# ishine/Prior-DiffuSE

Measured on AMD Instinct MI355X. Metric: enhanced-audio sec/sec (RTF), 6-step fast sampling, B=32, higher is better.
Workload: dtype f16x2; 1 GPU; B=32 x 4 s 16 kHz utterances per GPU, [B,2,401,161] spectrograms, GCRN prior + DiffUNet1 6-step sampling, STFT..ISTFT, seeded random weights; global_batch=32, frames=401, parallelism=batch-shard x1, graph=True, streams_per_gpu=1, batches_in_flight=3

## Files before the change

prior-diffuse_amd/csrc/gconv4.hip:

```cpp
#include <hip/hip_runtime.h>
#include <stdint.h>
#include <stdio.h>
#include <stdlib.h>

#include "pdse.h"
#include "pdse_internal.h"

#include "gconv_common.h"

#ifndef G4_CH
#define G4_CH 3
#endif

__device__ __forceinline__ void glds16_g4(const void* g, void* l) {
  __builtin_amdgcn_global_load_lds((const __attribute__((address_space(1))) void*)g, (__attribute__((address_space(3))) void*)l,
                                   16, 0, 0);
}

__device__ __forceinline__ float g4_load(const float* sbase, const unsigned byte_off) {
  float v;
  asm volatile("global_load_dword %0, %1, %2" : "=v"(v) : "v"(byte_off), "s"(sbase) : "memory");
  return v;
}
typedef float g4_f32x4 __attribute__((ext_vector_type(4)));
__device__ __forceinline__ g4_f32x4 g4_load16(const float* sbase, const unsigned byte_off) {
  g4_f32x4 v;
  asm volatile("global_load_dwordx4 %0, %1, %2" : "=v"(v) : "v"(byte_off), "s"(sbase) : "memory");
  return v;
}
template <bool BLK>
struct g4_raw {
  float v[G4_CH][8];
  __device__ __forceinline__ float get(const int i, const int e) const { return v[i][e]; }
};
template <>
struct g4_raw<true> {
  g4_f32x4 v[G4_CH][2];
  __device__ __forceinline__ float get(const int i, const int e) const { return v[i][e >> 2][e & 3]; }
};
__device__ __forceinline__ void g4_landed(g4_raw<false>& raw) {
#pragma unroll
  for (int i = 0; i < G4_CH; ++i)
#pragma unroll
    for (int e = 0; e < 8; ++e) asm volatile("" : "+v"(raw.v[i][e]));
}
__device__ __forceinline__ void g4_landed(g4_raw<true>& raw) {
#pragma unroll
  for (int i = 0; i < G4_CH; ++i)
#pragma unroll
    for (int e = 0; e < 2; ++e) asm volatile("" : "+v"(raw.v[i][e]));
}

typedef unsigned u32x4 __attribute__((ext_vector_type(4)));
__device__ __forceinline__ void g4_lds_read3(const unsigned addr, u32x4 (&a)[3]) {
  asm volatile("ds_read_b128 %0, %3\n\tds_read_b128 %1, %3 offset:1024\n\tds_read_b128 %2, %3 offset:2048"
               : "=&v"(a[0]), "=&v"(a[1]), "=&v"(a[2])
               : "v"(addr)
               : "memory");
}
__device__ __forceinline__ void g4_lds_read3(const unsigned addr, u32x4 (&a)[2]) {
  asm volatile("ds_read_b128 %0, %2\n\tds_read_b128 %1, %2 offset:1024" : "=&v"(a[0]), "=&v"(a[1]) : "v"(addr) : "memory");
}
__device__ __forceinline__ void g4_lds_read3(const unsigned addr, u32x4 (&a)[1]) {
  asm volatile("ds_read_b128 %0, %1" : "=&v"(a[0]) : "v"(addr) : "memory");
}
template <int N, int NP>
__device__ __forceinline__ void g4_lds_wait(u32x4 (&a)[N][NP]) {
  asm volatile("s_waitcnt lgkmcnt(0)" ::: "memory");
#pragma unroll
  for (int i = 0; i < N; ++i)
#pragma unroll
    for (int p = 0; p < NP; ++p) asm volatile("" : "+v"(a[i][p]));
}
__device__ __forceinline__ f32x16 g4_mfma6(const u32x4 (&a)[3], const uint4 (&b)[3], f32x16 acc) {
  const uint4 a1 = make_uint4(a[0][0], a[0][1], a[0][2], a[0][3]), a2 = make_uint4(a[1][0], a[1][1], a[1][2], a[1][3]),
              a3 = make_uint4(a[2][0], a[2][1], a[2][2], a[2][3]);
  acc = mfma_bf16(a1, b[2], acc);
  acc = mfma_bf16(a3, b[0], acc);
  acc = mfma_bf16(a2, b[1], acc);
  acc = mfma_bf16(a1, b[1], acc);
  acc = mfma_bf16(a2, b[0], acc);
  acc = mfma_bf16(a1, b[0], acc);
  return acc;
}
__device__ __forceinline__ f32x16 g4_mfma6(const u32x4 (&a)[2], const uint4 (&b)[2], f32x16 acc) {
  const uint4 a1 = make_uint4(a[0][0], a[0][1], a[0][2], a[0][3]), a2 = make_uint4(a[1][0], a[1][1], a[1][2], a[1][3]);
  acc = mfma_f16(a2, b[0], acc);
  acc = mfma_f16(a1, b[1], acc);
  acc = mfma_f16(a1, b[0], acc);
  return acc;
}
__device__ __forceinline__ f32x16 g4_mfma6(const u32x4 (&a)[1], const uint4 (&b)[1], f32x16 acc) {
  return mfma_bf16(make_uint4(a[0][0], a[0][1], a[0][2], a[0][3]), b[0], acc);
}
__device__ __forceinline__ uint32_t g4_pack_bf16(const float a, const float b) {
  typedef float f32x2 __attribute__((ext_vector_type(2)));
  typedef __bf16 bf16x2 __attribute__((ext_vector_type(2)));
  const f32x2 v = {a, b};
  union { bf16x2 h; uint32_t u; } c;
  c.h = __builtin_convertvector(v, bf16x2);
  return c.u;
}
__device__ __forceinline__ void g4_split(const float (&x)[8], uint4 (&b)[3]) { split8(x, b[0], b[1], b[2]); }
__device__ __forceinline__ void g4_split(const float (&x)[8], uint4 (&b)[2]) { split8h(x, pow2i(PDSE_F16_ACT_EXP), b[0], b[1]); }
__device__ __forceinline__ void g4_split(const float (&x)[8], uint4 (&b)[1]) {
  b[0] = make_uint4(g4_pack_bf16(x[0], x[1]), g4_pack_bf16(x[2], x[3]), g4_pack_bf16(x[4], x[5]), g4_pack_bf16(x[6], x[7]));
}

struct g4_chunk {
  int s, tap, cb0, n, kb0;
};

__device__ long long* g_trace4 = nullptr;

template <int EPI, int MT, bool BLK, int NP = 3>
__global__ __launch_bounds__(512, 2) void gconv4_kernel(const pdse_gconv_desc d) {
  constexpr int FB = 64 * NP;
#ifdef PDSE_DIAG
  long long* const trace = g_trace4;
#else
  long long* const trace = nullptr;
#endif
  const long long c_start = trace ? clock64() : 0;
  long long c_req = 0, c_cmp = 0, c_bar = 0;
  constexpr bool DUAL = (EPI != PDSE_EPI_LINEAR);
  constexpr int NBR = DUAL ? 2 : 1, FR = NBR * MT;
  extern __shared__ uint4 ring[];
  const unsigned ring_base = (unsigned)(uintptr_t)ring;
  const int tid = threadIdx.x;
  const int lane = tid & 63, wave = tid >> 6;
  const int col = lane & 31, h = lane >> 5;
// ... 156 lines not shown
#pragma unroll
      for (int r = 0; r < 16; ++r) {
        acc0[m][r] *= us;
        if (DUAL) acc1[m][r] *= us;
      }
  }
  gconv_epilogue<EPI, MT>(d, tail_from_desc(d), acc0, acc1, b, t, j, pvalid, lane, h, mt0, mtiles);
  if (trace && lane == 0) {
    long long* q = trace + ((size_t)((blockIdx.z * gridDim.y + blockIdx.y) * gridDim.x + blockIdx.x) * 8 + wave) * 8;
    q[0] = c_pro - c_start;
    q[1] = c_req;
    q[2] = c_cmp;
    q[3] = c_bar;
    q[4] = nch;
    q[5] = clock64() - c_loop;
    q[6] = clock64() - c_start;
  }
}

template <int EPI, int MT, bool BLK, int NP>
static int launch4b(const pdse_gconv_desc* d, hipStream_t s, const int mtiles) {
  const int P = d->Tout * d->Fout;
  const dim3 grid(((P + 31) / 32 + 7) / 8, d->B, (mtiles + MT - 1) / MT), block(512);
  constexpr int FR = (EPI == PDSE_EPI_LINEAR ? 1 : 2) * MT;
  const size_t lds = (size_t)2 * G4_CH * FR * 64 * NP * sizeof(uint4);
  static unsigned long long attr_mask = 0;
  if (lds > 64 * 1024 && pdse_lds_attr((const void*)gconv4_kernel<EPI, MT, BLK, NP>, &attr_mask, "gconv4 lds attribute")) return 1;
  static const bool tracing = PDSE_DIAG_ENV("PDSE_G4_TRACE") != nullptr;
  static long long* tbuf = nullptr;
  const size_t nw = (size_t)grid.x * grid.y * grid.z * 8;
  if (tracing) {
    if (!tbuf) {
      (void)hipMalloc(&tbuf, (size_t)1 << 24);
      (void)hipMemcpyToSymbol(HIP_SYMBOL(g_trace4), &tbuf, sizeof(tbuf));
    }
    (void)hipMemsetAsync(tbuf, 0, nw * 64, s);
  }
  hipLaunchKernelGGL((gconv4_kernel<EPI, MT, BLK, NP>), grid, block, lds, s, *d);
  if (tracing && nw * 64 <= ((size_t)1 << 24)) {
    (void)hipStreamSynchronize(s);
    long long* h = (long long*)malloc(nw * 64);
    (void)hipMemcpy(h, tbuf, nw * 64, hipMemcpyDeviceToHost);
    double sum[7] = {0};
    for (size_t i = 0; i < nw; ++i)
      for (int k = 0; k < 7; ++k) sum[k] += (double)h[i * 8 + k];
    fprintf(stderr, "gconv4 trace EPI %d MT %d taps %d cin %d+%d cout %d %dx%d grid %ux%ux%u: prologue %.0f | per chunk: request %.0f compute %.0f barrier %.0f | chunks %.1f | epilogue %.0f total %.0f\n",
            EPI, MT, d->ntaps, d->in0.C, d->in1.C, d->Cout, d->Tout, d->Fout, grid.x, grid.y, grid.z, sum[0] / nw, sum[1] / sum[4], sum[2] / sum[4], sum[3] / sum[4],
            sum[4] / nw, sum[5] / nw, sum[6] / nw);
    free(h);
  }
  return pdse_check_launch("gconv4");
}

template <int EPI, int MT>
static int launch4(const pdse_gconv_desc* d, hipStream_t s, const int mtiles) {
  if (d->korder == 5)
    return d->in0.blk ? launch4b<EPI, MT, true, 2>(d, s, mtiles) : launch4b<EPI, MT, false, 2>(d, s, mtiles);
  if (d->korder == 4)
    return d->in0.blk ? launch4b<EPI, MT, true, 1>(d, s, mtiles) : launch4b<EPI, MT, false, 1>(d, s, mtiles);
  return d->in0.blk ? launch4b<EPI, MT, true, 3>(d, s, mtiles) : launch4b<EPI, MT, false, 3>(d, s, mtiles);
}

static int check4(const pdse_gconv_desc* d) {
  const bool two = d->in1.C > 0;
  const long long span0 = 4 * ((long long)d->B * d->in0.sb + 40ll * d->in0.sc), span1 = two ? 4 * ((long long)d->B * d->in1.sb + 40ll * d->in1.sc) : 0;
  auto blk_ok = [](const pdse_src& x) {
    return x.blk == 0 || (x.blk == 8 && !((x.sb | x.sc | x.st | x.sf) & 3) && (reinterpret_cast<uintptr_t>(x.ptr) & 15) == 0);
  };
  if (!blk_ok(d->in0) || (two && !blk_ok(d->in1)) || (two && d->in0.blk != d->in1.blk)) {
    pdse_set_error("gconv4: a channel-blocked source has blk = 8, strides in multiples of 4 floats and a 16-byte aligned base; "
                   "two sources are both blocked or both plain");
    return 1;
  }
  if (!(d->epi == PDSE_EPI_LINEAR || d->epi == PDSE_EPI_GLU) || (d->in0.C & 15) || (d->in1.C & 15) || d->in0.C == 0 || d->cin1 ||
      d->xf_mode != 0 || d->padrow != nullptr || d->ntaps > 12 || span0 >= (1ll << 32) || span1 >= (1ll << 32) ||
      (d->epi == PDSE_EPI_GLU && !d->w1) || (d->korder == 5 && (d->wexp < -40 || d->wexp > 40))) {
    pdse_set_error("gconv4: split-bf16 GEMM convolutions need LINEAR / GLU, channel counts in multiples of 16, <= 12 taps, "
                   "no load transform / pad row, 32-bit gather offsets");
    return 1;
  }
  return 0;
}

int pdse_gconv4_launch(const pdse_gconv_desc* d, hipStream_t s) {
  if (check4(d)) return 1;
  const int mtiles = (d->Cout + 31) / 32;
  if (d->epi == PDSE_EPI_GLU) return mtiles >= 2 ? launch4<PDSE_EPI_GLU, 2>(d, s, mtiles) : launch4<PDSE_EPI_GLU, 1>(d, s, mtiles);
  if (mtiles >= 4) return launch4<PDSE_EPI_LINEAR, 4>(d, s, mtiles);
  if (mtiles >= 2) return launch4<PDSE_EPI_LINEAR, 2>(d, s, mtiles);
  return launch4<PDSE_EPI_LINEAR, 1>(d, s, mtiles);
}

template <int MT, bool BLK>
__global__ __launch_bounds__(512, 2) void gconv4_pair_kernel(const pdse_gconv_desc d, const pdse_gconv_desc e) {
  constexpr int NP = 2, FB = 64 * NP;
  constexpr int FR = 2 * MT, FR2 = 2 * FR;
  extern __shared__ uint4 ring[];
  const unsigned ring_base = (unsigned)(uintptr_t)ring;
  const int tid = threadIdx.x;
  const int lane = tid & 63, wave = tid >> 6;
  const int col = lane & 31, h = lane >> 5;
  const int b = blockIdx.y;
  const int P = d.Tout * d.Fout;
  const int p = (blockIdx.x * 8 + wave) * 32 + col;
  const bool pvalid = p < P;
  const int t = pvalid ? p / d.Fout : 0;
  const int j = pvalid ? p - t * d.Fout : 0;
  const int mtiles = (d.Cout + 31) >> 5;
  const int mt0 = blockIdx.z * MT;

  const int cbn0 = d.in0.C >> 4, cbn1 = d.in1.C >> 4;
  const int cps0 = (cbn0 + G4_CH - 1) / G4_CH, cps1 = (cbn1 + G4_CH - 1) / G4_CH;
  const int nch0 = d.ntaps * cps0, nch = nch0 + d.ntaps * cps1;

  auto uni = [](const int v) { return __builtin_amdgcn_readfirstlane(v); };
  auto decode = [&](const int ci) {
    g4_chunk c;
    c.s = uni(ci >= nch0);
    const int q = c.s ? ci - nch0 : ci, cps = c.s ? cps1 : cps0, cbn = c.s ? cbn1 : cbn0;
    c.tap = uni(q / cps);
    c.cb0 = uni((q - c.tap * cps) * G4_CH);
    c.n = uni(min(G4_CH, cbn - c.cb0));
    c.kb0 = uni((c.s ? d.ntaps * cbn0 : 0) + c.tap * cbn + c.cb0);
    return c;
  };
  auto dma = [&](const g4_chunk& c, const int buf) {
    const int nf = c.tap == 0 ? FR2 : FR;
    const int kb1 = (c.s ? cbn0 : 0) + c.cb0;
    const int npieces = c.n * nf * NP;
    for (int pc = __builtin_amdgcn_readfirstlane(wave); pc < npieces; pc += 8) {
      const int i = pc / (nf * NP), rem = pc - i * (nf * NP), f = rem / NP, part = rem - f * NP;
      const bool odd = f >= FR;
      const int g = odd ? f - FR : f, br = g / MT, m = g - br * MT;
      if (mt0 + m < mtiles) {
        const float* const w = odd ? (br ? e.w1 : e.w0) : (br ? d.w1 : d.w0);
        const uint4* src = reinterpret_cast<const uint4*>(w) + ((size_t)((odd ? kb1 : c.kb0) + i) * mtiles + mt0 + m) * FB + part * 64 + lane;
        glds16_g4(src, ring + ((buf * G4_CH + i) * FR2 + f) * FB + part * 64);
      }
    }
  };
  auto gather = [&](const g4_chunk& c, g4_raw<BLK>& raw, bool& inb) {
    const bool s1 = c.s != 0;
    const float* const sptr = s1 ? d.in1.ptr : d.in0.ptr;
    const int64_t ssb = s1 ? d.in1.sb : d.in0.sb, ssc = s1 ? d.in1.sc : d.in0.sc, sst = s1 ? d.in1.st : d.in0.st,
                  ssf = s1 ? d.in1.sf : d.in0.sf;
    int dt = 0, df = 0;
#pragma unroll
    for (int k = 0; k < 12; ++k) {
      dt = c.tap == k ? d.tap_dt[k] : dt;
      df = c.tap == k ? d.tap_df[k] : df;
    }
    const int tin = t + dt, fin = j * d.sf_in + df;
    inb = pvalid && fin >= 0 && fin < d.Fin && tin >= 0 && tin < d.Tin;
    if constexpr (BLK) {
      const unsigned off = 4u * (unsigned)((inb ? (int64_t)b * ssb + (int64_t)tin * sst + (int64_t)fin * ssf : 0) + (int64_t)h * ssc);
#pragma unroll
      for (int i = 0; i < G4_CH; ++i) {
        if (i < c.n) {
          const float* base = sptr + (int64_t)(2 * (c.cb0 + i)) * ssc;
          raw.v[i][0] = g4_load16(base, off);
          raw.v[i][1] = g4_load16(base + 4, off);
        }
      }
    } else {
      const unsigned off = 4u * (unsigned)((inb ? (int64_t)b * ssb + (int64_t)tin * sst + (int64_t)fin * ssf : 0) + (int64_t)(8 * h) * ssc);
#pragma unroll
      for (int i = 0; i < G4_CH; ++i) {
        if (i < c.n) {
          const float* base = sptr + (int64_t)(16 * (c.cb0 + i)) * ssc;
// ... 130 lines not shown
```

prior-diffuse_amd/nets.py:

```python
import ctypes as C

import numpy as np
import torch

from . import _lib as L
from . import packing as P

F0 = 161
BIG = 1 << 30

TAG_NONE, TAG_EPS_BLOCK, TAG_EPS_CONV1, TAG_TCM, TAG_PRIOR, TAG_LSTM, TAG_SIGNAL, TAG_EW = range(8)


class WeightBank:

    def __init__(self):
        self.items = {}
        self.keep = []
        self.owners = []

    def token(self, obj):
        if obj is None:
            return None
        for i, o in enumerate(self.owners):
# ... 154 lines not shown
        f["wlc"], f["wrc"] = up16(P.pack_s3_chain(chain["wlc"])), up16(P.pack_s3_chain(chain["wrc"]))
        f["blc"], f["brc"], f["bc2"] = up(chain["blc"]), up(chain["brc"]), up(chain["bc2"])
        f["wc2"] = up(np.asarray(chain["wc2"], np.float64).reshape(32)) if chain["C2"] == 1 else up16(P.pack_s3_chain(chain["wc2"]))
        nx = w.get("nx")
        if nx:
            for i, tl in enumerate(nx):
                if tl.get("bias") is not None:
                    f[("nx_bias", i)] = up(tl["bias"])
            f["nx_w"] = up16(np.stack([P.pack_s3_chain(tl["w"])[0] for tl in nx], 0))
        return f

    def _gconv_weights_s3g(self, w, ntaps, c0, c1):
        ctx = self.ctx
        up = lambda a: ctx.up(a).data_ptr()
        up16 = lambda a: ctx.up(np.ascontiguousarray(a).view(np.int16), np.int16).data_ptr()
        npl = self.gemm_planes
        qe = P.f16_wexp(*[w[k_] for k_ in ("wk0", "wk1") if w.get(k_) is not None]) if npl == 2 else 0
        f = {"korder": {3: 3, 1: 4, 2: 5}[npl], "ksteps": ntaps * (c0 + c1) // 2, "w0": up16(P.pack_s3_gemm(w["wk0"], ntaps, c0, c1, npl, qe)),
             "wexp": qe}
        if w.get("wk1") is not None:
            f["w1"] = up16(P.pack_s3_gemm(w["wk1"], ntaps, c0, c1, npl, qe))
        for k in ("bias0", "bias1"):
            if w.get(k) is not None:
                f[k] = up(w[k])
        if w.get("post") is not None:
            f["post_scale"], f["post_shift"] = up(w["post"][0]), up(w["post"][1])
        return f

    def _gconv_weights(self, w, ntaps, c0, c1, epi, cin1, pipelined_ok):
        ctx = self.ctx
        up = lambda a: ctx.up(a).data_ptr()
        f = {}
        xf = w.get("xf")
        xf_mode = 0
        if xf is not None:
            xf_mode = f["xf_mode"] = xf["mode"]
            f["xf_scale0"], f["xf_shift0"], f["xf_slope0"] = up(xf["scale0"]), up(xf["shift0"]), float(xf["slope0"])
            if xf["mode"] == 2:
                f["xf_scale1"], f["xf_shift1"], f["xf_slope1"] = up(xf["scale1"]), up(xf["shift1"]), float(xf["slope1"])
        wk0 = np.asarray(w["wk0"])
        wk1 = w.get("wk1")
        key = (epi, ntaps, c1 > 0, xf_mode)
        if P.v2_supported(*key, cin1) and pipelined_ok:
            rows = P.korder1_rows(ntaps, c0, c1, P.V2_CP[key])
            f["w0"], f["ksteps"], f["korder"] = up(P.pack_a4(wk0, rows)), len(rows) // 2, 1
            if wk1 is not None:
                f["w1"] = up(P.pack_a4(wk1, rows))
            if w.get("wk2") is not None:
                rows1 = P.korder1_rows(w["ntaps1"], c0, 0, P.V2_CP[key])
                f["w2"], f["w3"] = up(P.pack_a4(w["wk2"], rows1)), up(P.pack_a4(w["wk3"], rows1))
                f["ksteps1"] = len(rows1) // 2
        else:
            w0 = P.pack_a(wk0)
            f["w0"], f["ksteps"] = up(w0), w0.shape[1]
            if wk1 is not None:
                f["w1"] = up(P.pack_a(wk1))
        for k in ("bias0", "bias1"):
            if w.get(k) is not None:
                f[k] = up(w[k])
        if w.get("post") is not None:
            f["post_scale"], f["post_shift"] = up(w["post"][0]), up(w["post"][1])
        chain = w.get("chain")
        if chain is not None:
            f["C2"] = chain["C2"]
            f["wlc"], f["wrc"] = up(P.pack_chain(chain["wlc"])), up(P.pack_chain(chain["wrc"]))
            f["blc"], f["brc"] = up(chain["blc"]), up(chain["brc"])
            f["wc2"] = up(np.asarray(chain["wc2"], np.float64).reshape(32)) if chain["C2"] == 1 else up(P.pack_chain(chain["wc2"]))
            f["bc2"] = up(chain["bc2"])
        nx = w.get("nx")
        if nx:
            packs = []
            for i, tl in enumerate(nx):
                wn = np.asarray(tl["w"], np.float64)
                packs.append(np.concatenate([P.pack_chain(wn[:, :32]), P.pack_chain(wn[:, 32:])], 0))
                if tl.get("bias") is not None:
                    f[("nx_bias", i)] = up(tl["bias"])
            f["nx_w"] = up(np.stack(packs, 0))
        return f

    def gconv(self, *, in0, in1=None, Tin, Fin, taps, sf_in, W, Cout, bias0=None, bias0_sb=0,
              bias1=None, bias1_sb=0, epi=L.EPI_LINEAR, act=L.ACT_NONE, act_slope=0.0,
              padrow=None, padrow_sb=0, padrow_off=0, cin1=False, resid=None, out,
              out_strides, out_off=0, out_cr=1, B, Tout, Fout, tag=TAG_NONE, bias0_off=0, phase1=None, nx=None,
              bias1_off=0, bias_t0=None, label="gconv", s3=False, s3g=False, has_xf=False):
        ctx = self.ctx
        d = L.GconvDesc()
        d.in0 = in0
        d.in1 = in1 if in1 is not None else L.Src(0, 0, 0, 0, 0, 0, 0)
        d.Tin, d.Fin = Tin, Fin
        d.padrow, d.padrow_sb = Ctx.ptr(padrow, padrow_off), padrow_sb
        ttaps = tuple((int(a), int(b)) for a, b in taps)
        tkey = ("taps", ttaps)
        tp = ctx.bank.items.get(tkey)
        if tp is None:
            ctx._banking += 1
            tp = ctx.bank.items[tkey] = ctx.up(P.taps_array(ttaps), np.int32)
            ctx._banking -= 1
        d.taps, d.ntaps, d.sf_in = tp.data_ptr(), len(ttaps), sf_in
        for i, (dt_, df_) in enumerate(ttaps[:12]):
            d.tap_dt[i], d.tap_df[i] = dt_, df_
        d.cin1 = 1 if cin1 else 0
        c0, c1 = d.in0.C, d.in1.C
        pipelined_ok = padrow is None and not self.force_generic
        s3 = bool(s3) and pipelined_ok and epi == L.EPI_BIGLU and (
            ((c0, c1) == (32, 0) and len(ttaps) in (4, 6)) or ((c0, c1, len(ttaps)) == (2, 2, 10) and phase1 is None))
        s3g = (bool(s3g) and not s3 and pipelined_ok and epi in (L.EPI_LINEAR, L.EPI_GLU) and not cin1 and not has_xf
               and c0 > 0 and c0 % 16 == 0 and c1 % 16 == 0 and len(ttaps) <= 12)
        site = "%s:%d:%d:%d:%d:%d:%d:%d:%d" % (label, epi, len(ttaps), c0, c1, Cout, pipelined_ok, s3, s3g)
        if s3g:
            f = self.memo(site, lambda: self._gconv_weights_s3g(W(), len(ttaps), c0, c1))
        elif s3:
            f = self.memo(site, lambda: self._gconv_weights_s3(W(), len(ttaps), c0 + c1))
        else:
            f = self.memo(site, lambda: self._gconv_weights(W(), len(ttaps), c0, c1, epi, cin1, pipelined_ok))
        for k, v in f.items():
            if isinstance(k, tuple):
                d.nx_bias[k[1]] = v
            else:
                setattr(d, k, v)
        d.Cout = Cout
        if bias0 is not None:
            d.bias0 = Ctx.ptr(bias0, bias0_off)
        if bias1 is not None:
            d.bias1 = Ctx.ptr(bias1, bias1_off)
        d.bias0_sb, d.bias1_sb = bias0_sb, bias1_sb
        if bias_t0 is not None:
            d.bias0_t0, d.bias1_t0 = Ctx.ptr(bias_t0[0], bias_t0[1]), Ctx.ptr(bias_t0[0], bias_t0[2])
        d.epi, d.act, d.act_slope = epi, act, float(act_slope)
        if phase1 is not None and d.korder in (1, 2):
            d.p1mask, d.Fout1 = phase1["mask"], phase1["Fout1"]
        elif phase1 is not None and d.korder == 5 and epi == L.EPI_GLU:
            d.p1mask, d.Fout1 = phase1["mask"], phase1["Fout1"]
        if nx is not None:
            tiles = nx["tiles"]
            d.nx_n, d.nx_keep, d.nx_row0 = len(tiles), 1 if nx.get("keep") else 0, nx.get("row0", -1)
            for i, tl in enumerate(tiles):
                if tl.get("bias") is not None:
                    d.nx_bias[i] = Ctx.ptr(tl["bias"], tl.get("bias_off", 0))
                d.nx_bias_sb[i] = tl.get("bias_sb", 0)
                d.nx_out[i] = Ctx.ptr(tl["out"])
                d.nx_sb[i], d.nx_sc[i], d.nx_st[i], d.nx_sf[i] = tl["strides"]
                d.nx_off[i] = tl.get("off", 0)
                d.nx_add[i] = Ctx.ptr(tl.get("add"))
        d.resid = Ctx.ptr(resid)
        d.out = Ctx.ptr(out)
        d.out_sb, d.out_sc_hi, d.out_sc_lo, d.out_st, d.out_sf = out_strides
        d.out_off, d.out_cr = out_off, out_cr
        d.B, d.Tout, d.Fout = B, Tout, Fout
        self.add(d, tag)
        return d


def nchw(C_, T, F):
    return C_ * T * F, T * F, F, 1


def nchw_out(C_, T, F):
    return C_ * T * F, T * F, 0, F, 1


def nc8(C_, T, F):
    return C_ * T * F, T * F * 8, F * 8, 8


def nc8_out(C_, T, F):
    return C_ * T * F, T * F * 8, 1, F * 8, 8


class EpsNetPlan(PlanBase):

    ENC_F = [161, 79, 39, 19, 9, 4]
    fused_tcm = True
    chain_conv1 = True
    compose_stage1 = True
    split_bf16 = True
    split_tcm = True
    plane_h = True
    tcm_stack = True
    parity_planes = True
    planes = 2
    TCM_F16 = True
    NSLOT = 20

    def __init__(self, ctx, sd, B, T, time_cond=True, nsteps=1, plan=None, table=None, with_pre=None, split_bf16=None,
                 planes=None, plane_h=None, exclusive=False, frames=None):
        with_pre = time_cond if with_pre is None else with_pre
        if split_bf16 is not None:
            self.split_bf16 = bool(split_bf16)
        if planes is not None:
            if int(planes) not in (1, 2, 3):
                raise ValueError("planes is 3 (bf16x3), 2 (f16x2) or 1 (bf16 mode)")
            self.planes = int(planes)
        if plane_h is not None:
            self.plane_h = bool(plane_h)
        if self.planes == 1:
            self.plane_h = True
        self.tcm_planes = 3 if (self.planes == 2 and not self.TCM_F16) else self.planes
        self.use_tcm_stack = bool(self.tcm_stack and exclusive)
        self.frames = frames
        if frames is not None and (self.force_generic or not self.fused_tcm):
            raise ValueError("exact ragged batches need a fused TCM form (csrc/tcm.hip, csrc/tcm2.hip): the three-launch form has no frames table")
        self.sd = sd
        ok = (self.split_bf16 and self.chain_conv1 and self.compose_stage1 and time_cond and with_pre and not self.force_generic
              and all(float(P._np(sd[k])[0]) <= 1.0 for k in sd if k.endswith(".weight") and P._np(sd[k]).shape == (1,)))
        if not ok:
            if self.planes == 1:
                raise ValueError("bf16 mode needs the chained split-bf16 DiffUNet1 path (PReLU slopes <= 1)")
            self.plane_h = False
            if self.planes == 2:
                self.planes = self.tcm_planes = 3
        super().__init__(ctx, plan, ns=(ctx.bank.token(sd), bool(time_cond), bool(with_pre), self.fused_tcm, self.chain_conv1,
                                        self.compose_stage1, self.split_bf16, self.split_tcm,
                                        ctx.bank.token(table), str(self.plane_h), self.planes, self.parity_planes))
        self.sd, self.B, self.T, self.time_cond, self.nsteps = sd, B, T, time_cond, nsteps
        self.with_pre = with_pre
# ... 622 lines not shown
                nx = dict(keep=False, row0=0, tiles=tiles)
            if chained and k == 1 and self.compose_stage1:
                Fin = self._biconvglu_composed(step, src_x, src_i, o, ostr, nx)
            else:
                Fin = self._biconvglu(step, k, src_x, src_i, Fin, o, ostr, H=Hc, do_conv1=(k == 1 or not chained), nx=nx)
            if chained:
                Hc, Hn = Hn, Hc
            src_x, src_i = self.src(o, 64, *nchw(64, T, Fin)), None
        cur, nxt = self.en[4], self.tcm_a
        names = [("TCMs.%d.residual%d" % (i, j + 1), dil) for i in range(3) for j, dil in enumerate((1, 2, 4, 8, 16, 32))]
        if self.force_generic or not self.fused_tcm:
            for p, dil in names:
                self._residual(p, dil, cur, nxt)
                cur, nxt = nxt, (self.tcm_b if nxt is self.tcm_a else self.tcm_a)
        elif self.split_bf16 and self.split_tcm:
            hcur, hnxt = self.tcm_hs
            self._residual_split(None, 1, cur, None, None, hcur, names[0][0], mode=1)
            self._tcm_stack = [] if self.use_tcm_stack else None
            for n, (p, dil) in enumerate(names):
                p_next = names[n + 1][0] if n + 1 < len(names) else None
                self._residual_split(p, dil, cur, nxt, hcur, hnxt, p_next)
                cur, nxt = nxt, (self.tcm_b if nxt is self.tcm_a else self.tcm_a)
                hcur, hnxt = hnxt, hcur
            if self._tcm_stack:
                sd_ = L.Tcm2sDesc()
                for n, blk in enumerate(self._tcm_stack):
                    sd_.blk[n] = blk
                sd_.n = len(self._tcm_stack)
                sd_.flags, sd_.status = self.tcm_flags.data_ptr(), self.tcm_status.data_ptr()
                self.add(sd_, TAG_TCM)
            self._tcm_stack = None
        else:
            hcur, hnxt = self.tcm_h, self.tcm_g
            self._tcm_conv1(names[0][0], cur, hcur)
            for n, (p, dil) in enumerate(names):
                p_next = names[n + 1][0] if n + 1 < len(names) else None
                self._residual_fused(p, dil, cur, nxt, hcur, hnxt, p_next)
                cur, nxt = nxt, (self.tcm_b if nxt is self.tcm_a else self.tcm_a)
                hcur, hnxt = hnxt, hcur
        tcm_out = cur
        if self._plane_stage("dec"):
            self._decoders_planes(step, tcm_out, out)
            return out
        for di, de in enumerate(("de_real", "de_imag")):
            in0 = self.src(tcm_out, 64, 256 * T, 4 * T, 1, T)
            Fin = 4
            Hc, Hn = self.H, self.H2
            for n, k in enumerate((5, 4, 3, 2, 1)):
                skip = self.en[k - 1]
                if k == 5:
                    in1 = self.src(skip, 64, 256 * T, 4 * T, 1, T)
                else:
                    in1 = self.src(skip, 64, *nchw(64, T, self.ENC_F[k]))
                p = "%s.de%d.0" % (de, k)
                if k > 1:
                    o, ooff = self.dec[n & 1], 0
                    fn = lambda Fo: nchw_out(64, T, Fo)
                    bn, pr = "%s.de%d.2" % (de, k), "%s.de%d.3.weight" % (de, k)
                else:
                    o, ooff = out, di * T * F0
                    fn = lambda Fo: nchw_out(2, T, Fo)
                    bn, pr = None, None
                nx = None
                if chained and k > 1:
                    Fo = 2 * (Fin - 1) + 3
                    wn = lambda de=de, k=k: self.w("%s.de%d.0.conv1.weight" % (de, k - 1))[:, :, 0, 0].T[:, :64]
                    nx = dict(keep=False, row0=-1, tiles=[dict(wfn=wn, bias=self.zero32, out=Hn, add=self.Pskip[di][k - 1],
                                                                strides=(32 * T * Fo, T * Fo, Fo, 2))])
                Fin = self._biconvtransglu(step, 5 + 5 * di + n, p, k, in0, in1, Fin, o, fn, bn, pr, out_off=ooff, H=Hc,
                                           do_conv1=(k == 5 or not chained), nx=nx)
                if chained:
                    Hc, Hn = Hn, Hc
                in0 = self.src(o, 64, *nchw(64, T, Fin))
        return out


class GcrnPlan(PlanBase):
    fused_last = True
    fused_glstm = True
    split_bf16 = True
    gemm_planes = 2
    block8 = True
    fuse_phases = True
    persist_lstm = True
    PERSIST_MAX_B = 4
    ENC_C = [2, 16, 32, 64, 128, 256]
    ENC_F = [161, 80, 39, 19, 9, 4]

    def __init__(self, ctx, sd, B, T, plan=None, split_bf16=None, exclusive=False, planes=None):
        if split_bf16 is not None:
            self.split_bf16 = bool(split_bf16)
        if planes is not None:
            if planes not in (1, 2, 3) or (planes in (1, 2) and not self.split_bf16):
                raise ValueError("planes is 3 (bf16x3), 2 (f16x2) or 1 (bf16 mode); the one- and two-plane forms run on the GEMM kernels (split_bf16)")
            self.gemm_planes = int(planes)
        self.persist = bool(self.persist_lstm and self.fused_glstm and exclusive and B <= self.PERSIST_MAX_B and not self.force_generic)
        self.exclusive = bool(exclusive)
        super().__init__(ctx, plan, ns=(ctx.bank.token(sd), self.fused_last, self.fused_glstm, self.split_bf16, self.block8, self.persist,
                                        self.gemm_planes))
        self.sd, self.B, self.T = sd, B, T
        a = ctx.alloc
        self.Bp = Bp = (B + 31) // 32 * 32
        self.status = None
        self.x = a(B, 2, T, F0)
        self.out = a(B, 2, T, F0)
        self.e = [a(B, self.ENC_C[i + 1], T, self.ENC_F[i + 1]) for i in range(5)]
        self.gx = a(2, T, 2048, Bp, zero=True)
        self.hT = a(2, 2, 512, Bp, zero=True)
        self.cst = a(2, 512, Bp, zero=True)
        self.y = a(B, T, 1024)
        if self.persist:
            bq = 1 << (B - 1).bit_length()
            self.gran = torch.zeros(4 * 1024 * bq, dtype=torch.int64, device=ctx.device)
            self.status = torch.zeros(4, dtype=torch.int32, device=ctx.device)
            ctx.keep += [self.gran, self.status]
        elif self.fused_glstm and not self.force_generic:
            self.hT2, self.cst2 = a(2, 2, 512, Bp, zero=True), a(2, 512, Bp, zero=True)
            self.gx2, self.part = a(2, 2, 2048, Bp, zero=True), a(2, 2, 64, Bp, 2, zero=True)
        else:
            self.yn = a(B, 1024, T)
        self.glstm = a(B, 256, T, 4)
        self.d = [a(B, 128, T, 9), a(B, 64, T, 19), a(B, 32, T, 39), a(B, 16, T, 80), a(B, 1, T, 161)]
        for i, t_ in enumerate(self.e):
            self.named("gcrn.e%d" % (i + 1), t_)
        self.named("gcrn.glstm", self.glstm)
        for i, t_ in enumerate(self.d[:4]):
            self.named("gcrn.d%d" % (5 - i), t_)
        self.named("gcrn.x", self.x)

    def w(self, k):
        return P._np(self.sd[k])

    def _nchw(self, t, blocked):
        if blocked and self.split_bf16 and not self.force_generic and self.block8:
            B, C_, T, F = t.shape
            return t.view(B, C_ // 8, T, F, 8).permute(0, 1, 4, 2, 3).reshape(B, C_, T, F)
        return t

    def enc_out(self, k):
        return self._nchw(self.e[k - 1], k >= 2)

    def glstm_out(self):
        return self._nchw(self.glstm, True)

    def _lstm_layer(self, layer, xproj_src_fn, y_su, y_sg):
        B, T, Bp = self.B, self.T, self.Bp
        for g in range(2):
            p = "glstm.%s.%d." % (layer, g)
            in0, Tin, Fin, taps, wk_fn, Tout, Fout, ost, osf = xproj_src_fn(g)
            self.gconv(in0=in0, Tin=Tin, Fin=Fin, taps=taps, sf_in=1, Cout=2048,
                       W=lambda p=p, wk_fn=wk_fn: dict(wk0=wk_fn(self.w(p + "weight_ih_l0")),
                                                       bias0=self.w(p + "bias_ih_l0") + self.w(p + "bias_hh_l0")),
                       out=self.gx, out_strides=(1, Bp, 0, ost, osf), out_off=g * T * 2048 * Bp, B=B, Tout=Tout, Fout=Fout,
                       tag=TAG_PRIOR, label=p + "ih", s3g=self.split_bf16)

        def pack_whh():
            return P.pack_lstm_whh([self.w("glstm.%s.%d.weight_hh_l0" % (layer, g)) for g in range(2)])

        d = L.LstmDesc()
        d.gx, d.whh = self.gx.data_ptr(), self.upw(layer + ".whh", pack_whh).data_ptr()
        d.hT, d.cst, d.y = self.hT.data_ptr(), self.cst.data_ptr(), self.y.data_ptr()
        d.y_sb, d.y_st, d.y_su, d.y_sg = T * 1024, 1024, y_su, y_sg
        d.B, d.Bp, d.T, d.H, d.G = B, Bp, T, 512, 2
        self.add(d, TAG_LSTM)

    def _glstm_natural(self):
        per = lambda key: [self.w("glstm.%s" % (key % g)) for g in range(2)]
        return (per("lstm_list1.%d.weight_hh_l0"), per("lstm_list2.%d.weight_ih_l0"), per("lstm_list2.%d.bias_ih_l0"),
                per("lstm_list2.%d.bias_hh_l0"), per("lstm_list2.%d.weight_hh_l0"), self.w("glstm.ln1.weight"), self.w("glstm.ln1.bias"))

    def _glstm_wavefront(self, proj1):
        B, T, Bp = self.B, self.T, self.Bp
        for g in range(2):
            p = "glstm.lstm_list1.%d." % g
            in0, Tin, Fin, taps, wk_fn, Tout, Fout, ost, osf = proj1(g)
            self.gconv(in0=in0, Tin=Tin, Fin=Fin, taps=taps, sf_in=1, Cout=2048,
                       W=lambda p=p, wk_fn=wk_fn: dict(wk0=wk_fn(self.w(p + "weight_ih_l0")),
                                                       bias0=self.w(p + "bias_ih_l0") + self.w(p + "bias_hh_l0")),
                       out=self.gx, out_strides=(2048, 1, 0, ost, osf), out_off=g * T * 2048 * Bp, B=B, Tout=Tout, Fout=Fout,
                       tag=TAG_PRIOR, label=p + "ih", s3g=self.split_bf16)

        def pack():
            return {k: self.ctx.up(v).data_ptr() for k, v in P.pack_glstm_wavefront(*self._glstm_natural()).items()}

        d = L.GlstmDesc()
        for k, v in self.memo("glstm.wavefront", pack).items():
            setattr(d, k, v)
        d.gx1, d.gx2, d.part = self.gx.data_ptr(), self.gx2.data_ptr(), self.part.data_ptr()
        d.hT1, d.cst1, d.hT2, d.cst2 = self.hT.data_ptr(), self.cst.data_ptr(), self.hT2.data_ptr(), self.cst2.data_ptr()
        d.y, d.y_sb, d.y_st, d.y_su, d.y_sg = self.y.data_ptr(), T * 1024, 1024, 1, 512
        d.B, d.Bp, d.T, d.H, d.G, d.eps = B, Bp, T, 512, 2, 1e-5
        d.slices = 2 if self.exclusive else 1
        self.add(d, TAG_LSTM)

    def _glstm_persistent(self, proj1):
        B, T, Bp = self.B, self.T, self.Bp
        for g in range(2):
            p = "glstm.lstm_list1.%d." % g
            in0, Tin, Fin, taps, wk_fn, Tout, Fout, ost, osf = proj1(g)
            self.gconv(in0=in0, Tin=Tin, Fin=Fin, taps=taps, sf_in=1, Cout=2048,
                       W=lambda p=p, wk_fn=wk_fn: dict(wk0=wk_fn(self.w(p + "weight_ih_l0")),
                                                       bias0=self.w(p + "bias_ih_l0") + self.w(p + "bias_hh_l0")),
                       out=self.gx, out_strides=(2048, 1, 0, ost, osf), out_off=g * T * 2048 * Bp, B=B, Tout=Tout, Fout=Fout,
                       tag=TAG_PRIOR, label=p + "ih", s3g=self.split_bf16)

        def pack():
            return {k: self.ctx.up(v).data_ptr() for k, v in P.pack_glstm_persistent(*self._glstm_natural()).items()}

        d = L.GlstmpDesc()
        for k, v in self.memo("glstm.persistent", pack).items():
            setattr(d, k, v)
        d.gx1, d.gran, d.status = self.gx.data_ptr(), self.gran.data_ptr(), self.status.data_ptr()
        d.y, d.y_sb, d.y_st, d.y_su, d.y_sg = self.y.data_ptr(), T * 1024, 1024, 1, 512
        d.B, d.Bp, d.T, d.H, d.G, d.eps = B, Bp, T, 512, 2, 1e-5
        self.add(d, TAG_LSTM)

    def _ln(self, name, out_t, osb, os_hi, os_lo, os_t, r, blk=0):
        d = L.LnDesc()
        d.blk = blk
        d.in_, d.out = self.y.data_ptr(), out_t.data_ptr()
        d.gamma = self.upw(name + ".g", lambda: self.w(name + ".weight")).data_ptr()
        d.beta = self.upw(name + ".b", lambda: self.w(name + ".bias")).data_ptr()
        d.osb, d.os_hi, d.os_lo, d.os_t = osb, os_hi, os_lo, os_t
        d.B, d.T, d.N, d.r, d.eps = self.B, self.T, 1024, r, 1e-5
        self.add(d, TAG_PRIOR)

    def build(self, x=None, out=None):
        B, T, Bp = self.B, self.T, self.Bp
        x = self.x if x is None else x
        out = self.out if out is None else out
        blk = self.split_bf16 and not self.force_generic and self.block8

        def lay(k_is_blocked, C_, Fq):
            if k_is_blocked:
                return nc8(C_, T, Fq), nc8_out(C_, T, Fq), 8
            return nchw(C_, T, Fq), nchw_out(C_, T, Fq), 1

        src = self.src(x, 2, *nchw(2, T, F0))
        e_lay = [lay(blk and k >= 2, self.ENC_C[k], self.ENC_F[k]) for k in range(1, 6)]
        for k in range(1, 6):
            ci, co, Fin, Fout = self.ENC_C[k - 1], self.ENC_C[k], self.ENC_F[k - 1], self.ENC_F[k]
            kk, taps = P.conv_taps(1, 3, 0)
            p = "conv%d" % k
            ist, ost_, ocr = e_lay[k - 1]
            self.gconv(in0=src, Tin=T, Fin=Fin, taps=taps, sf_in=2, Cout=co, epi=L.EPI_GLU, act=L.ACT_ELU,
                       W=lambda p=p, k=k, kk=kk: dict(wk0=P.conv_kmat(self.sd[p + ".conv1.weight"], kk),
                                                      wk1=P.conv_kmat(self.sd[p + ".conv2.weight"], kk),
                                                      bias0=self.w(p + ".conv1.bias"), bias1=self.w(p + ".conv2.bias"),
                                                      post=P.bn_fold(self.sd, "bn%d" % k)),
                       out=self.e[k - 1], out_strides=ost_, out_cr=ocr, B=B, Tout=T, Fout=Fout, tag=TAG_PRIOR, label=p,
                       s3g=self.split_bf16)
            src = self.src(self.e[k - 1], co, *ist, blk=8 if ocr == 8 else 0)

        def proj1(g):
            wk = lambda Wih: np.concatenate([Wih[:, f::4].T for f in range(4)], axis=0)
            s = self.src(self.e[4], 128, *e_lay[4][0], off=128 * g * T * 4, blk=8 if blk else 0)
            return s, T, 4, [(0, f) for f in range(4)], wk, T, 1, 2048 * Bp, 0

        if self.persist:
            self._glstm_persistent(proj1)
        elif self.fused_glstm and not self.force_generic:
            self._glstm_wavefront(proj1)
        else:
            self._lstm_layer("lstm_list1", proj1, y_su=2, y_sg=1)
            self._ln("glstm.ln1", self.yn, 1024 * T, T, 0, 1, 1)

            def proj2(g):
                s = self.src(self.yn, 512, 1024 * T, T, 0, 1, off=512 * g * T)
                return s, 1, T, [(0, 0)], (lambda Wih: Wih.T), 1, T, 0, 2048 * Bp

            self._lstm_layer("lstm_list2", proj2, y_su=1, y_sg=512)
        if blk:
            self._ln("glstm.ln2", self.glstm, 256 * T * 4, T * 4 * 8, 8, 4 * 8, 4, blk=8)
        else:
            self._ln("glstm.ln2", self.glstm, 256 * T * 4, T * 4, 1, 4, 4)

        dec = [(5, 512, 128), (4, 256, 64), (3, 128, 32), (2, 64, 16), (1, 32, 1)]
        for br in (1, 2):
            in0 = self.src(self.glstm, 256, *(nc8(256, T, 4) if blk else nchw(256, T, 4)), blk=8 if blk else 0)
            in1 = self.src(self.e[4], 256, *e_lay[4][0], blk=8 if blk else 0)
            Fin = 4
            for n, (k, ci, co) in enumerate(dec):
                p = "conv%d_t_%d" % (k, br)
                Fout = 2 * (Fin - 1) + 3 + (1 if k == 2 else 0)
                if k == 1 and self.fused_last and not self.force_generic:
                    def last(p=p, br=br):
                        up = lambda a: self.ctx.up(a).data_ptr()
# ... 486 lines not shown
```

Baseline: 9445 audio_s/s.

## Add flat position-tiled split-bf16 GEMM kernel for LSTM input projections

Adds a new gconv4 kernel variant that tiles over flattened batch*time positions (Fout == 1), with 8 output M-tiles per block and double-buffered weight DMA into LDS. It is used for the GLSTM input projections (Cout 2048) when the flat_proj flag is set. The aim is to raise weight reuse and avoid the per-batch grid layout, which leaves tiles poorly filled when Fout is 1. In exchange it needs more LDS and registers per block, which may lower occupancy. The g4_raw helper is templated on its channel count so the new kernel can share it.

```diff
diff --git a/prior-diffuse_amd/csrc/gconv4.hip b/prior-diffuse_amd/csrc/gconv4.hip
--- a/prior-diffuse_amd/csrc/gconv4.hip
+++ b/prior-diffuse_amd/csrc/gconv4.hip
@@ -28,25 +28,27 @@
   asm volatile("global_load_dwordx4 %0, %1, %2" : "=v"(v) : "v"(byte_off), "s"(sbase) : "memory");
   return v;
 }
-template <bool BLK>
+template <bool BLK, int CH = G4_CH>
 struct g4_raw {
-  float v[G4_CH][8];
+  float v[CH][8];
   __device__ __forceinline__ float get(const int i, const int e) const { return v[i][e]; }
 };
-template <>
-struct g4_raw<true> {
-  g4_f32x4 v[G4_CH][2];
+template <int CH>
+struct g4_raw<true, CH> {
+  g4_f32x4 v[CH][2];
   __device__ __forceinline__ float get(const int i, const int e) const { return v[i][e >> 2][e & 3]; }
 };
-__device__ __forceinline__ void g4_landed(g4_raw<false>& raw) {
-#pragma unroll
-  for (int i = 0; i < G4_CH; ++i)
+template <int CH>
+__device__ __forceinline__ void g4_landed(g4_raw<false, CH>& raw) {
+#pragma unroll
+  for (int i = 0; i < CH; ++i)
 #pragma unroll
     for (int e = 0; e < 8; ++e) asm volatile("" : "+v"(raw.v[i][e]));
 }
-__device__ __forceinline__ void g4_landed(g4_raw<true>& raw) {
-#pragma unroll
-  for (int i = 0; i < G4_CH; ++i)
+template <int CH>
+__device__ __forceinline__ void g4_landed(g4_raw<true, CH>& raw) {
+#pragma unroll
+  for (int i = 0; i < CH; ++i)
 #pragma unroll
     for (int e = 0; e < 2; ++e) asm volatile("" : "+v"(raw.v[i][e]));
 }
@@ -369,9 +371,193 @@
   return 0;
 }
 
+#define G4F_MT 8
+#ifndef G4F_CH
+#define G4F_CH 2
+#endif
+#ifndef G4F_HR
+#define G4F_HR 4
+#endif
+template <bool BLK>
+__global__ __launch_bounds__(512, 2) void gconv4_flat_kernel(const pdse_gconv_desc d) {
+  constexpr int NP = 2, FB = 64 * NP, MT = G4F_MT, HR = G4F_HR, CH = G4F_CH;
+  extern __shared__ uint4 ring[];
+  const unsigned ring_base = (unsigned)(uintptr_t)ring;
+  const int tid = threadIdx.x;
+  const int lane = tid & 63, wave = tid >> 6;
+  const int col = lane & 31, h = lane >> 5;
+  const int p = (blockIdx.x * 8 + wave) * 32 + col;
+  const bool pvalid = p < d.B * d.Tout;
+  const int b = pvalid ? p / d.Tout : 0;
+  const int t = pvalid ? p - b * d.Tout : 0;
+  const int mtiles = (d.Cout + 31) >> 5;
+  const int mt0 = blockIdx.y * MT;
+
+  const int cbn = d.in0.C >> 4;
+  const int cps = (cbn + CH - 1) / CH;
+  const int nch = d.ntaps * cps;
+
+  auto uni = [](const int v) { return __builtin_amdgcn_readfirstlane(v); };
+  auto decode = [&](const int ci) {
+    g4_chunk c;
+    c.s = 0;
+    c.tap = uni(ci / cps);
+    c.cb0 = uni((ci - c.tap * cps) * CH);
+    c.n = uni(min(CH, cbn - c.cb0));
+    c.kb0 = uni(c.tap * cbn + c.cb0);
+    return c;
+  };
+  auto dma = [&](const g4_chunk& c, const int buf) {
+    const int npieces = c.n * MT * NP;
+    for (int pc = __builtin_amdgcn_readfirstlane(wave); pc < npieces; pc += 8) {
+      const int i = pc / (MT * NP), rem = pc - i * (MT * NP), m = rem / NP, part = rem - m * NP;
+      if (mt0 + m < mtiles) {
+        const uint4* src = reinterpret_cast<const uint4*>(d.w0) + ((size_t)(c.kb0 + i) * mtiles + mt0 + m) * FB + part * 64 + lane;
+        glds16_g4(src, ring + ((buf * CH + i) * MT + m) * FB + part * 64);
+      }
+    }
+  };
+  auto gather = [&](const g4_chunk& c, g4_raw<BLK, CH>& raw, bool& inb) {
+    const float* const sptr = d.in0.ptr;
+    const int64_t ssb = d.in0.sb, ssc = d.in0.sc, sst = d.in0.st, ssf = d.in0.sf;
+    int dt = 0, df = 0;
+#pragma unroll
+    for (int k = 0; k < 12; ++k) {
+      dt = c.tap == k ? d.tap_dt[k] : dt;
+      df = c.tap == k ? d.tap_df[k] : df;
+    }
+    const int tin = t + dt, fin = df;
+    inb = pvalid && fin >= 0 && fin < d.Fin && tin >= 0 && tin < d.Tin;
+    const int64_t pos = inb ? (int64_t)b * ssb + (int64_t)tin * sst + (int64_t)fin * ssf : 0;
+    if constexpr (BLK) {
+      const unsigned off = 4u * (unsigned)(pos + (int64_t)h * ssc);
+#pragma unroll
+      for (int i = 0; i < CH; ++i) {
+        if (i < c.n) {
+          const float* base = sptr + (int64_t)(2 * (c.cb0 + i)) * ssc;
+          raw.v[i][0] = g4_load16(base, off);
+          raw.v[i][1] = g4_load16(base + 4, off);
+        }
+      }
+    } else {
+      const unsigned off = 4u * (unsigned)(pos + (int64_t)(8 * h) * ssc);
+#pragma unroll
+      for (int i = 0; i < CH; ++i) {
+        if (i < c.n) {
+          const float* base = sptr + (int64_t)(16 * (c.cb0 + i)) * ssc;
+#pragma unroll
+          for (int e = 0; e < 8; ++e) raw.v[i][e] = g4_load(base + (int64_t)e * ssc, off);
+        }
+      }
+    }
+  };
+
+  f32x16 acc[MT];
+#pragma unroll
+  for (int m = 0; m < MT; ++m)
+#pragma unroll
+    for (int r = 0; r < 16; ++r) acc[m][r] = 0.f;
+
+  const bool elu = uni(d.in0.act == PDSE_ACT_ELU) != 0;
+  auto compute = [&](const g4_chunk& c, const g4_raw<BLK, CH>& raw, const bool inb, const int buf) {
+    u32x4 af[HR][NP];
+    const unsigned wa0 = ring_base + (unsigned)((((buf * CH) * MT) * FB + lane) * 16);
+#pragma unroll
+    for (int f = 0; f < HR; ++f) g4_lds_read3(wa0 + f * (FB * 16), af[f]);
+#pragma unroll
+    for (int i = 0; i < CH; ++i) {
+      if (i < c.n) {
+        float x[8];
+#pragma unroll
+        for (int e = 0; e < 8; ++e) x[e] = inb ? raw.get(i, e) : 0.f;
+        if (elu) {
+#pragma unroll
+          for (int e = 0; e < 8; ++e) x[e] = x[e] < 0.f ? fast_exp(x[e]) - 1.0f : x[e];
+        }
+        uint4 bp[NP];
+        g4_split(x, bp);
+        g4_lds_wait(af);
+        const bool more = i + 1 < c.n;
+        const unsigned wi = ring_base + (unsigned)((((buf * CH + i) * MT) * FB + lane) * 16);
+        const unsigned wn = wi + MT * FB * 16;
+#pragma unroll
+        for (int rd = 0; rd < MT / HR; ++rd) {
+          if (rd) g4_lds_wait(af);
+#pragma unroll
+          for (int f = 0; f < HR; ++f) {
+            acc[rd * HR + f] = g4_mfma6(af[f], bp, acc[rd * HR + f]);
+            if (rd + 1 < MT / HR) g4_lds_read3(wi + ((rd + 1) * HR + f) * (FB * 16), af[f]);
+            else if (i + 1 < CH && more) g4_lds_read3(wn + f * (FB * 16), af[f]);
+          }
+        }
+      }
+    }
+  };
+
+  g4_raw<BLK, CH> rawA, rawB;
+  bool inbA = false, inbB = false;
+  g4_chunk cA = decode(0), cB = cA;
+  gather(cA, rawA, inbA);
+  dma(cA, 0);
+  __syncthreads();
+  g4_landed(rawA);
+  for (int ci = 0; ci < nch; ci += 2) {
+    const bool hasB = ci + 1 < nch;
+    if (hasB) {
+      cB = decode(ci + 1);
+      gather(cB, rawB, inbB);
+      dma(cB, 1);
+    }
+    compute(cA, rawA, inbA, 0);
+    __syncthreads();
+    if (!hasB) break;
+    g4_landed(rawB);
+    if (ci + 2 < nch) {
+      cA = decode(ci + 2);
+      gather(cA, rawA, inbA);
+      dma(cA, 0);
+    }
+    compute(cB, rawB, inbB, 1);
+    __syncthreads();
+    g4_landed(rawA);
+  }
+  const float us = pow2i(-(PDSE_F16_ACT_EXP + d.wexp));
+#pragma unroll
+  for (int m = 0; m < MT; ++m)
+#pragma unroll
+    for (int r = 0; r < 16; ++r) acc[m][r] *= us;
+  gconv_epilogue<PDSE_EPI_LINEAR, MT>(d, tail_from_desc(d), acc, acc, b, t, 0, pvalid, lane, h, mt0, mtiles);
+}
+
+static bool wants_flat(const pdse_gconv_desc* d) { return d->korder == 5 && d->epi == PDSE_EPI_LINEAR && d->w2 == nullptr && d->ksteps1 == 1; }
+
+static int check4f(const pdse_gconv_desc* d) {
+  if (d->Fout != 1 || d->in1.C != 0 || (long long)d->B * d->Tout >= (1ll << 31) - 256) {
+    pdse_set_error("gconv4: flat position tiles (ksteps1 1 on a korder 5 LINEAR launch) need Fout == 1, one source "
+                   "and B * Tout < 2^31 - 256");
+    return 1;
+  }
+  return 0;
+}
+
+template <bool BLK>
+static int launch4f(const pdse_gconv_desc* d, hipStream_t s, const int mtiles) {
+  const long long npos = (long long)d->B * d->Tout;
+  const dim3 grid((unsigned)((npos + 255) / 256), (mtiles + G4F_MT - 1) / G4F_MT), block(512);
+  const size_t lds = (size_t)2 * G4F_CH * G4F_MT * 64 * 2 * sizeof(uint4);
+  static unsigned long long attr_mask = 0;
+  if (lds > 64 * 1024 && pdse_lds_attr((const void*)gconv4_flat_kernel<BLK>, &attr_mask, "gconv4 flat lds attribute")) return 1;
+  hipLaunchKernelGGL((gconv4_flat_kernel<BLK>), grid, block, lds, s, *d);
+  return pdse_check_launch("gconv4 flat");
+}
+
 int pdse_gconv4_launch(const pdse_gconv_desc* d, hipStream_t s) {
   if (check4(d)) return 1;
   const int mtiles = (d->Cout + 31) / 32;
+  if (wants_flat(d)) {
+    if (check4f(d)) return 1;
+    return d->in0.blk ? launch4f<true>(d, s, mtiles) : launch4f<false>(d, s, mtiles);
+  }
   if (d->epi == PDSE_EPI_GLU) return mtiles >= 2 ? launch4<PDSE_EPI_GLU, 2>(d, s, mtiles) : launch4<PDSE_EPI_GLU, 1>(d, s, mtiles);
   if (mtiles >= 4) return launch4<PDSE_EPI_LINEAR, 4>(d, s, mtiles);
   if (mtiles >= 2) return launch4<PDSE_EPI_LINEAR, 2>(d, s, mtiles);
diff --git a/prior-diffuse_amd/nets.py b/prior-diffuse_amd/nets.py
--- a/prior-diffuse_amd/nets.py
+++ b/prior-diffuse_amd/nets.py
@@ -260,7 +260,7 @@
               bias1=None, bias1_sb=0, epi=L.EPI_LINEAR, act=L.ACT_NONE, act_slope=0.0,
               padrow=None, padrow_sb=0, padrow_off=0, cin1=False, resid=None, out,
               out_strides, out_off=0, out_cr=1, B, Tout, Fout, tag=TAG_NONE, bias0_off=0, phase1=None, nx=None,
-              bias1_off=0, bias_t0=None, label="gconv", s3=False, s3g=False, has_xf=False):
+              bias1_off=0, bias_t0=None, label="gconv", s3=False, s3g=False, has_xf=False, flat=False):
         ctx = self.ctx
         d = L.GconvDesc()
         d.in0 = in0
@@ -309,6 +309,8 @@
             d.p1mask, d.Fout1 = phase1["mask"], phase1["Fout1"]
         elif phase1 is not None and d.korder == 5 and epi == L.EPI_GLU:
             d.p1mask, d.Fout1 = phase1["mask"], phase1["Fout1"]
+        elif flat and d.korder == 5 and epi == L.EPI_LINEAR:
+            d.ksteps1 = 1
         if nx is not None:
             tiles = nx["tiles"]
             d.nx_n, d.nx_keep, d.nx_row0 = len(tiles), 1 if nx.get("keep") else 0, nx.get("row0", -1)
@@ -1097,6 +1099,7 @@
     gemm_planes = 2
     block8 = True
     fuse_phases = True
+    flat_proj = True
     persist_lstm = True
     PERSIST_MAX_B = 4
     ENC_C = [2, 16, 32, 64, 128, 256]
@@ -1167,7 +1170,7 @@
                        W=lambda p=p, wk_fn=wk_fn: dict(wk0=wk_fn(self.w(p + "weight_ih_l0")),
                                                        bias0=self.w(p + "bias_ih_l0") + self.w(p + "bias_hh_l0")),
                        out=self.gx, out_strides=(1, Bp, 0, ost, osf), out_off=g * T * 2048 * Bp, B=B, Tout=Tout, Fout=Fout,
-                       tag=TAG_PRIOR, label=p + "ih", s3g=self.split_bf16)
+                       tag=TAG_PRIOR, label=p + "ih", s3g=self.split_bf16, flat=self.flat_proj and Fout == 1)
 
         def pack_whh():
             return P.pack_lstm_whh([self.w("glstm.%s.%d.weight_hh_l0" % (layer, g)) for g in range(2)])
@@ -1193,7 +1196,7 @@
                        W=lambda p=p, wk_fn=wk_fn: dict(wk0=wk_fn(self.w(p + "weight_ih_l0")),
                                                        bias0=self.w(p + "bias_ih_l0") + self.w(p + "bias_hh_l0")),
                        out=self.gx, out_strides=(2048, 1, 0, ost, osf), out_off=g * T * 2048 * Bp, B=B, Tout=Tout, Fout=Fout,
-                       tag=TAG_PRIOR, label=p + "ih", s3g=self.split_bf16)
+                       tag=TAG_PRIOR, label=p + "ih", s3g=self.split_bf16, flat=self.flat_proj and Fout == 1)
 
         def pack():
             return {k: self.ctx.up(v).data_ptr() for k, v in P.pack_glstm_wavefront(*self._glstm_natural()).items()}
@@ -1217,7 +1220,7 @@
                        W=lambda p=p, wk_fn=wk_fn: dict(wk0=wk_fn(self.w(p + "weight_ih_l0")),
                                                        bias0=self.w(p + "bias_ih_l0") + self.w(p + "bias_hh_l0")),
                        out=self.gx, out_strides=(2048, 1, 0, ost, osf), out_off=g * T * 2048 * Bp, B=B, Tout=Tout, Fout=Fout,
-                       tag=TAG_PRIOR, label=p + "ih", s3g=self.split_bf16)
+                       tag=TAG_PRIOR, label=p + "ih", s3g=self.split_bf16, flat=self.flat_proj and Fout == 1)
 
         def pack():
             return {k: self.ctx.up(v).data_ptr() for k, v in P.pack_glstm_persistent(*self._glstm_natural()).items()}
```

After: 9533 audio_s/s (median of 6 runs). No clear change (+0.9%).
